# caomw/3DFeatureMatcher

Measured on AMD Instinct MI355X. Metric: matched+triangulated+normal-optimised keypoints/sec; HBM GB/s vs roofline, higher is better.
Workload: dtype f64

## Files before the change

### 3dfeaturematcher_amd/__init__.py

```python
from __future__ import annotations

import ctypes
import os

import numpy as np

_HERE = os.path.dirname(os.path.abspath(__file__))
LIB_PATH = os.environ.get("FM3D_LIB") or os.path.join(_HERE, "libfm3d.so")

FM3D_OK = 0
ERR_INVALID, ERR_HIP, ERR_UNSUPPORTED, ERR_NOMEM, ERR_PARSE, ERR_NAN_PLANE = -1, -2, -3, -4, -5, -6
FEAT_SURF, FEAT_ORB, FEAT_SIFT, FEAT_FAST, FEAT_STAR, FEAT_BRISK, FEAT_FREAK, FEAT_MSER, FEAT_OTHER = 0, 1, 2, 3, 4, 5, 6, 7, -1
DESC_F32, DESC_U8, DESC_BITS = 0, 1, 2
ST_OK, ST_NO_PIXELS, ST_ABORT_BBOX, ST_ABORT_PIX1, ST_ABORT_PIX2, ST_NAN_PLANE, ST_NAN_NORMAL = range(7)

EXPORTS = (
    "fm3d_settings_default", "fm3d_settings_load", "fm3d_settings_lookup", "fm3d_ctx_create", "fm3d_ctx_destroy", "fm3d_last_error",
    "fm3d_ctx_set_stream", "fm3d_knn2", "fm3d_match_nndr", "fm3d_setg12", "fm3d_g12_from_poses",
    "fm3d_camera2_from_g12", "fm3d_set_g12", "fm3d_get_camera2", "fm3d_triangulate", "fm3d_set_images",
    "fm3d_get_pyramid_level", "fm3d_optimize_normals", "fm3d_pipeline_upload", "fm3d_pipeline_run",
    "fm3d_records_download", "fm3d_pyrdown", "fm3d_neighborhood", "fm3d_undistort", "fm3d_version",
    "fm3d_gravity", "fm3d_features_frames", "fm3d_patch_size", "fm3d_export_patches", "fm3d_square_neighborhoods",
    "fm3d_circular_neighborhoods", "fm3d_surf_detect", "fm3d_surf_compute", "fm3d_extract_descriptors_from_patches", "fm3d_extract_descriptors_from_patches_any", "fm3d_pipeline_run_dlt", "fm3d_pipeline_dlt_download", "fm3d_pipeline_run_ncc",
    "fm3d_pipeline_ncc_download",
# ... 96 lines not shown
                     ("octave", "<i4"), ("class_id", "<i4")])
RECORD = np.dtype([("queryIdx", "<i4"), ("trainIdx", "<i4"), ("distance", "<f4"), ("status", "<i4"),
                   ("point", "<f8", (3,)), ("normal", "<f8", (3,))])


class LMStats(ctypes.Structure):
    _fields_ = [("points_in", ctypes.c_int64), ("points_kept", ctypes.c_int64), ("evaluations", ctypes.c_int64),
                ("pixel_evaluations", ctypes.c_int64), ("drops", ctypes.c_int64 * 8), ("kernel_ms", ctypes.c_double),
                ("groups", ctypes.c_int64), ("passes", ctypes.c_int64), ("cycles_terms", ctypes.c_int64),
                ("cycles_chain", ctypes.c_int64), ("cycles_control", ctypes.c_int64), ("cycles_total", ctypes.c_int64),
                ("wall_ticks_sum", ctypes.c_int64), ("wall_ticks_max", ctypes.c_int64),
                ("wall_clock_khz", ctypes.c_int64), ("class_passes", ctypes.c_int64 * 4),
                ("class_cycles", ctypes.c_int64 * 4), ("last_group_start_ticks", ctypes.c_int64),
                ("last_group_end_ticks", ctypes.c_int64), ("cycles_wait", ctypes.c_int64),
                ("chain_rounds", ctypes.c_int64), ("chain_chunks", ctypes.c_int64),
                ("queue_empty_ticks", ctypes.c_int64)]

    def as_dict(self):
        d = {k: getattr(self, k) for k, _ in self._fields_}
        for k in ("drops", "class_passes", "class_cycles"):
            d[k] = list(d[k])
        return d


class PipelineStats(ctypes.Structure):
    _fields_ = [("queries", ctypes.c_int64), ("trains", ctypes.c_int64), ("matches", ctypes.c_int64),
                ("inliers", ctypes.c_int64), ("kept", ctypes.c_int64), ("match_ms", ctypes.c_double),
                ("nndr_ms", ctypes.c_double), ("triangulate_ms", ctypes.c_double), ("pyramid_ms", ctypes.c_double),
                ("lm_ms", ctypes.c_double), ("total_ms", ctypes.c_double), ("lm", LMStats)]

    def as_dict(self):
        d = {k: getattr(self, k) for k, _ in self._fields_ if k != "lm"}
        d["lm"] = self.lm.as_dict()
        return d

# ... 1500 lines not shown
```

### 3dfeaturematcher_amd/csrc/fm3d_ctx.h

```cpp
#pragma once

#include <hip/hip_runtime.h>

#include <cstdint>
#include <cstdlib>
#include <string>
#include <vector>

#include "fm3d.h"
#include "fm3d_algebra.h"
#include "fm3d_kernels.h"

namespace fm3d_host {

inline bool poison_word(uint32_t* word) {
    const char* e = getenv("FM3D_DEBUG_POISON");
    if (!e || !e[0]) return false;
    *word = (uint32_t)strtoul(e, nullptr, 0);
    return true;
}
inline void poison_host(void* p, size_t n, uint32_t word) {
    uint8_t* b = (uint8_t*)p;
    for (size_t i = 0; i < n; i++) b[i] = (uint8_t)(word >> (8 * (i & 3)));
}
// ... 68 lines not shown
        uint32_t word;
        if (poison_word(&word)) poison_host(p, n, word);
        return hipSuccess;
    }
};
using DevBuf = Buf<DeviceMem>;
using HostBuf = Buf<PinnedMem>;

constexpr size_t kGuard(int w) { return (size_t)4 * w + 64; }
constexpr int kColStride(int h) { return (h + 2 + 63) / 64 * 64; }
constexpr size_t kColBytes(int w, int h) { return (size_t)(w + 2) * kColStride(h) + 64; }

struct PipeSmall {
    int32_t cnt[4];
    unsigned long long prob[2];
    unsigned long long lm[26];
};

struct KnnWork {
    DevBuf cq, ct;
    DevBuf q8, t8;
    DevBuf partIdx, partKey;
    DevBuf pairs;
    DevBuf idx, key, fkey;
};

enum class PairState { Idle, Full, MemberFront, DltFront, Ncc, Verified, DltVerified };

enum class Need { Idle, StagedIdle, Full, Dlt, Ncc, Verified, DltVerified };

enum Ev {
// ... 177 lines not shown
```

### 3dfeaturematcher_amd/csrc/fm3d_kernels.h

```cpp
#pragma once

#include <hip/hip_runtime.h>
#include <stdint.h>

#include "fm3d.h"
#include "fm3d_device.h"

#ifndef FM3D_RAY_AOS
#define FM3D_RAY_AOS 1
#endif

namespace fm3d {

struct LevelDesc {
    const uint8_t* img1;
    const uint8_t* img2;
    int w, h;
    const uint8_t* img2t;
    int hs;
};

struct ProjConst {
    double R[9], t[3];
    Camera cam;
// ... 37 lines not shown
    double* normals_;
    int* status_;
    int* info_;
    int* nfev_;
    int* mdat_;
    unsigned long long* statEval;
    unsigned long long* statPix;
    long long maxIter;
    long long maxTicks;
    int* overflow;
    int coop;
    int safe;
    unsigned long long* statPass;
    int nProb;
    const LMProblem* prob;
};
constexpr int kLMMaxProblems = 4;

constexpr int kLMRunning = 0x100;

constexpr int kLM2Slots = 15;
constexpr int kLM2Ring = 8;
constexpr int kLM2Threads = 64 * (kLM2Slots + 1);
template <bool MULTI, bool TREE, bool COLS>
__global__ void lm2_kernel(LMParams p);

struct KnnOut {
    int* idx;
    int* key;
    float* fkey;
};

// ... 375 lines not shown
```

### 3dfeaturematcher_amd/csrc/fm3d_lm.cpp

```cpp
#include <cmath>
#include <cstdlib>
#include <cstring>
#include <vector>

#include "fm3d_ctx.h"

using fm3d::LevelDesc;

using namespace fm3d_host;

namespace fm3d_host {

void fill_lm_cycles(const fm3d_ctx* c, const unsigned long long* cnt, fm3d_lm_stats* st) {
    st->groups = c->lmGroups;
    st->passes = (int64_t)cnt[3];
    st->cycles_terms = (int64_t)cnt[4];
    st->cycles_chain = (int64_t)cnt[5];
    st->cycles_control = (int64_t)cnt[6];
    st->cycles_total = (int64_t)cnt[7];
    st->wall_ticks_sum = (int64_t)cnt[8];
    st->wall_ticks_max = (int64_t)cnt[9];
    st->wall_clock_khz = c->wallKhz;
    for (int k = 0; k < 4; k++) {
        st->class_passes[k] = (int64_t)cnt[10 + k];
        st->class_cycles[k] = (int64_t)cnt[14 + k];
    }
    st->last_group_start_ticks = (int64_t)(cnt[18] - cnt[20]);
    st->last_group_end_ticks = (int64_t)(cnt[19] - cnt[20]);
    st->cycles_wait = (int64_t)cnt[24];
    st->chain_rounds = (int64_t)cnt[21];
    st->chain_chunks = (int64_t)cnt[22];
    st->queue_empty_ticks = cnt[25] ? (int64_t)(cnt[25] - cnt[20]) : 0;
}

fm3d::Camera lm_camera(const fm3d::Camera& cam) {
    fm3d::Camera k = cam;
    if (k.cx == 0.) k.cx = 0.;
    if (k.cy == 0.) k.cy = 0.;
    return k;
}

int lm_groups(fm3d_ctx* c, const void* kptr, int slots, long Ptot, long* out) {
    long groups = c->s.lmWaves;
    if (groups <= 0) {
        int cus = 0, perCU = 0;
        HIPCHK(c, hipDeviceGetAttribute(&cus, hipDeviceAttributeMultiprocessorCount, c->device));
        HIPCHK(c, hipOccupancyMaxActiveBlocksPerMultiprocessor(&perCU, kptr, fm3d::kLM2Threads, 0));
// ... 48 lines not shown
        if (q != c && (q->device != c->device || q->s.pyramids != levels || q->s.pixelsRay != c->s.pixelsRay ||
                       std::memcmp(&q->cam, &c->cam, sizeof(c->cam)) != 0 || q->s.boundWidth != c->s.boundWidth ||
                       q->s.boundHeight != c->s.boundHeight || q->s.zThresholdMax != c->s.zThresholdMax ||
                       q->s.epsilonLMMIN != c->s.epsilonLMMIN || q->s.lmReduction != c->s.lmReduction))
            return fail(c, FM3D_ERR_INVALID, "linked contexts need one device, camera and LM settings");
        const int P = src[j].P;
        HIPCHK(c, q->lmNormals.ensure((size_t)(P + 1) * 3 * sizeof(double)));
        HIPCHK(c, q->lmStatus.ensure((size_t)(P + 1) * sizeof(int)));
        HIPCHK(c, q->lmInfo.ensure((size_t)(P + 1) * 8 * sizeof(int)));
        HIPCHK(c, q->lmNfev.ensure((size_t)(P + 1) * 8 * sizeof(int)));
        HIPCHK(c, q->lmMdat.ensure((size_t)(P + 1) * sizeof(int)));
        HIPCHK(c, q->pcnt.ensure(64));
        Ptot += P;
    }
    HIPCHK(c, c->lmQueue.ensure(64 * sizeof(int)));
    HIPCHK(c, c->lmStat.ensure(256));
    if (c->s.lmReduction != 0 && c->s.lmReduction != 1)
        return fail(c, FM3D_ERR_INVALID, "lmReduction must be 0 (pixel order) or 1 (tree)");
    const bool tree = c->s.lmReduction != 0;
    const int slots = fm3d::kLM2Slots + (tree ? 1 : 0);
    bool multiPose = false;
    for (int j = 1; j < nProb; j++)
        multiPose |= std::memcmp(src[j].c->R2, src[0].c->R2, sizeof(c->R2)) != 0 ||
                     std::memcmp(src[j].c->t2, src[0].c->t2, sizeof(c->t2)) != 0;
    bool cols = true;
    for (int j = 0; j < nProb; j++) cols &= lm_prefers_cols(src[j].c);
    if (const char* lay = getenv("FM3D_LM_IMG2")) {
        if (!std::strcmp(lay, "rows")) cols = false;
        else if (!std::strcmp(lay, "cols")) cols = true;
        else if (std::strcmp(lay, "auto")) return fail(c, FM3D_ERR_INVALID, "FM3D_LM_IMG2 must be rows, cols or auto");
    }
// ... 78 lines not shown
    c->lmGroups = groups;
    {
        const long long perSlot = (Ptot + groups * slots - 1) / (groups * slots) + 1;
        p.maxIter = perSlot * (long long)(levels + 1) * 1600 + 10000;
        int khz = 0;
        if (hipDeviceGetAttribute(&khz, hipDeviceAttributeWallClockRate, c->device) != hipSuccess || khz <= 0) khz = 100000;
        const char* ms = getenv("FM3D_LM_MAX_SECONDS");
        const double secs = ms && atof(ms) > 0 ? atof(ms) : 300.;
        p.maxTicks = (long long)((double)khz * 1000. * secs);
        c->wallKhz = khz;
        const char* co = getenv("FM3D_LM_COOP");
        p.coop = co ? atoi(co) : 1;
        if (tree) p.coop = 0;
        const char* sf = getenv("FM3D_LM_SAFE");
        p.safe = sf ? atoi(sf) : 0;
    }
    {
        fm3d::LMReset rz{};
        rz.stat = c->lmStat.as<unsigned long long>();
        rz.queue = Ptot > 0 ? c->lmQueue.as<int>() : nullptr;
        rz.nProb = nProb;
        for (int j = 0; j < nProb; j++) {
            fm3d_ctx* q = src[j].c;
            rz.pcnt16[j] = q->pcnt.as<int>() + 4;
            rz.status[j] = q->lmStatus.as<int>();
            rz.info[j] = q->lmInfo.as<int>();
            rz.nfev[j] = q->lmNfev.as<int>();
            rz.P[j] = Ptot > 0 && src[j].P > 0 ? src[j].P : 0;
        }
        if (Ptot > 0) HIPCHK(c, hipEventRecord(e0, c->stream));
// ... 18 lines not shown
}

}

extern "C" {

int fm3d_optimize_normals(fm3d_ctx* c, double* points, int P, double* normals, int32_t* status, int32_t* info,
                          int32_t* nfev, int* nKept, fm3d_lm_stats* stats) {
    if (!c || !nKept || P < 0 || (P && (!points || !normals))) return fail(c, FM3D_ERR_INVALID, "bad argument");
    hipSetDevice(c->device);
    int r;
    if ((r = upload(c, c->pts, points, (size_t)P * 3 * sizeof(double)))) return r;
    if ((r = run_lm(c, P, nullptr, stats, c->ev[EV_LM_START], c->ev[EV_END]))) return r;
    std::vector<double> nrm((size_t)P * 3);
    std::vector<int> st(P), inf((size_t)P * 8), nf((size_t)P * 8);
    unsigned long long cnt[26] = {};
    if (P) {
        HIPCHK(c, hipMemcpyAsync(nrm.data(), c->lmNormals.p, nrm.size() * sizeof(double), hipMemcpyDeviceToHost, c->stream));
        HIPCHK(c, hipMemcpyAsync(st.data(), c->lmStatus.p, st.size() * sizeof(int), hipMemcpyDeviceToHost, c->stream));
        HIPCHK(c, hipMemcpyAsync(inf.data(), c->lmInfo.p, inf.size() * sizeof(int), hipMemcpyDeviceToHost, c->stream));
        HIPCHK(c, hipMemcpyAsync(nf.data(), c->lmNfev.p, nf.size() * sizeof(int), hipMemcpyDeviceToHost, c->stream));
        HIPCHK(c, hipMemcpyAsync(cnt, c->lmStat.p, sizeof(cnt), hipMemcpyDeviceToHost, c->stream));
    }
    HIPCHK(c, hipStreamSynchronize(c->stream));
    int overflow = 0;
    HIPCHK(c, hipMemcpy(&overflow, c->lmStat.as<unsigned long long>() + 2, sizeof(int), hipMemcpyDeviceToHost));
    if (overflow) return fail(c, FM3D_ERR_HIP, "LM kernel iteration guard tripped (internal error)");
    float ms = 0.f;
    if (P) hipEventElapsedTime(&ms, c->ev[EV_LM_START], c->ev[EV_END]);
    int kept = 0;
    bool nanPlane = false;
// ... 31 lines not shown
```

### 3dfeaturematcher_amd/csrc/fm3d_lm2.hip

```cpp
#include <hip/hip_runtime.h>
#include <float.h>
#include <stdint.h>

#include <type_traits>

#include "fm3d_device.h"
#include "fm3d_fastdiv.h"
#include "fm3d_kernels.h"
#include "fm3d_lmdif.h"

namespace fm3d {

namespace {

using namespace lmdif;

constexpr int kW = kLM2Slots;
constexpr int kWA = kW + 1;
constexpr int kE = 64;
constexpr int kR = kLM2Ring;
static_assert((kR & (kR - 1)) == 0, "ring depth: a power of two");
constexpr int kRow = kE + 2;
constexpr int kRS = (2 * kLM2Slots * kRow * 8 + 255) / 256 * 256 / 8;
#ifndef FM3D_EVAL_PIPE
#define FM3D_EVAL_PIPE 1
#endif

enum PassKind2 { Q_IDLE = 0, Q_INIT, Q_LEVEL, Q_EVAL, Q_QR1, Q_QR2, Q_QR3, Q_GRAM, Q_DONE };
enum SumKind { S_NONE = 0, S_ENORM, S_DOT };

typedef __attribute__((address_space(1))) double gdouble;
typedef __attribute__((address_space(1))) float gfloat;
typedef double d2v __attribute__((ext_vector_type(2)));
typedef __attribute__((address_space(1))) d2v gd2v;
typedef __attribute__((address_space(1))) int gint;
typedef __attribute__((address_space(1))) const long long gi64;
typedef __attribute__((address_space(1))) const uint8_t gu8;
// ... 23 lines not shown
    int pidx, m, L, i1ok, ekind, t0, q0, t1, bNaN;
};

struct PassOut2 {
    double nrm[2];
    double sum[2];
    double aqs1;
    double sq[2], g[3];
    int cnt, fail[2], ph3[2], i1fail, slow;
};

struct PassDesc {
    int nChunks, id;
    int kind[2];
    double agiant;
};

struct Slab {
    gdouble* RX;
    gdouble* RY;
    gfloat* I1;
    gfloat* DF;
    gfloat* DJ0;
    gfloat* DJ1;
    gint* KI;
};
template <int NS>
__device__ inline Slab slab_of(const LMParams& p, long gslot) {
    const size_t n = (size_t)p.nOffPad, G = (size_t)p.nWaves * NS;
    Slab s;
// ... 416 lines not shown
            }
        } else if (ps == Q_GRAM) {
            S.s.acnorm[0] = o.nrm[0];
            S.s.acnorm[1] = o.nrm[1];
            start_qr_tree(S, P, o);
        } else if (ps == Q_QR3) {
            const double tq1 = -o.sum[0] / S.usecond;
            finalize_qr(S, P, S.wa4s + S.usecond * tq1);
        }
    }
};

struct Shared {
    alignas(256) double ring[kR][kRS];
    int rowTag[kWA][kR];
    int consumed[kWA][2];
    int resultId[kWA][2];
    double result[kWA][2];
    Enorm chainEn[64];
    int done[kWA];
    int exited;
    int helper[kWA];
    int annSeq[kWA];
    int annBase[kWA], annId[kWA];
    int helpDone[kWA];
    int hfail[kWA][2], hph3[kWA][2];
    int hAtt[kWA], hSeen[kWA], hAnn[kWA];
    struct WaveStat {
        unsigned long long cnt[4], cyc[4], terms, ctl, wait, nPass, iter, t0;
    } ws[kWA];
// ... 51 lines not shown
    add(v1);
    add(v2);
    add(v3);
    return sum;
}

__device__ __forceinline__ int rfl(int v) { return __builtin_amdgcn_readfirstlane(v); }
__device__ __forceinline__ unsigned long long rfl_u64(unsigned long long v) {
    return ((unsigned long long)(unsigned)rfl((int)(v >> 32)) << 32) | (unsigned)rfl((int)v);
}
__device__ __forceinline__ const uint8_t* rfl_ptr(const uint8_t* q) {
    const unsigned long long v = (unsigned long long)q;
    return (const uint8_t*)(((unsigned long long)(unsigned)rfl((int)(v >> 32)) << 32) | (unsigned)rfl((int)v));
}

struct Producer {
    Shared* sh;
    int w, lane, me;
    int cmin;
    unsigned long long deadline;

    __device__ __forceinline__ void reserve(int c) {
        if (c >= cmin + kR) {
            cmin = rfl(min(lds_load_acq(&sh->consumed[w][0]), lds_load_acq(&sh->consumed[w][1])));
            if (c >= cmin + kR) {
                const long long c0 = clock64();
                do {
                    __builtin_amdgcn_s_sleep(1);
                    cmin = rfl(min(lds_load_acq(&sh->consumed[w][0]), lds_load_acq(&sh->consumed[w][1])));
                } while (c >= cmin + kR && wall_clock64() < deadline);
                const unsigned long long dt = clock64() - c0;
                if (lane == 0) sh->ws[me].wait += dt;
            }
        }
    }
    template <bool TWO = true>
    __device__ __forceinline__ void write(int c, double t0, double t1, int slowBits) {
        const int pos = c & (kR - 1);
        double* row0 = &sh->ring[pos][2 * w * kRow];
        row0[lane] = t0;
        if (TWO) row0[kRow + lane] = t1;
#if FM3D_TAG_NOWAIT
        __hip_atomic_store(&sh->rowTag[w][pos], (c << 2) | slowBits, __ATOMIC_RELAXED, __HIP_MEMORY_SCOPE_WORKGROUP);
#else
        __builtin_amdgcn_s_waitcnt(0xc07f);
        lds_store_rel(&sh->rowTag[w][pos], (c << 2) | slowBits);
#endif
    }
    template <bool TWO = true>
    __device__ __forceinline__ void put(int c, double t0, double t1, int slowBits) {
        reserve(c);
        write<TWO>(c, t0, t1, slowBits);
    }
#ifndef FM3D_SLOW_BRANCH
#define FM3D_SLOW_BRANCH 1
#endif
    template <bool TWO = true>
    __device__ __forceinline__ void write_terms(int c, double t0, double v0, bool slow0, double t1, double v1,
                                                bool slow1) {
#if FM3D_SLOW_BRANCH
        const int pos = c & (kR - 1);
        double* row0 = &sh->ring[pos][2 * w * kRow];
        row0[lane] = t0;
        if (TWO) row0[kRow + lane] = t1;
        int slowBits = 0;
        if (slow0 || (TWO && slow1)) {
            asm volatile("" ::: "memory");
            if (slow0) row0[lane] = v0;
            if (TWO && slow1) row0[kRow + lane] = v1;
            slowBits = (slow0 ? 1 : 0) | ((TWO && slow1) ? 2 : 0);
        }
        __builtin_amdgcn_s_waitcnt(0xc07f);
        lds_store_rel(&sh->rowTag[w][pos], (c << 2) | slowBits);
#else
        write<TWO>(c, slow0 ? v0 : t0, slow1 ? v1 : t1, (slow0 ? 1 : 0) | (slow1 ? 2 : 0));
#endif
    }
};

typedef __attribute__((address_space(4))) const ProjConst cProjConst;

__device__ __forceinline__ const cProjConst* proj_consts(const ProjConst* p) {
    int z;
    asm volatile("s_mov_b32 %0, 0" : "=s"(z));
    return (const cProjConst*)((const __attribute__((address_space(4))) char*)p + z);
}
__device__ __forceinline__ const cProjConst* proj_consts(const ProjConst* p, unsigned off) {
    unsigned z;
    asm volatile("s_mov_b32 %0, %1" : "=s"(z) : "s"(off));
    return (const cProjConst*)((const __attribute__((address_space(4))) char*)p + z);
}
// ... 94 lines not shown

__device__ __forceinline__ double chain_slow(int lane, double acc0, const double* row) {
    Enorm en = g_sh.chainEn[lane];
    en.s2 = acc0;
    for (int i = 0; i < kE; i++) en.add(row[i]);
    g_sh.chainEn[lane] = en;
    return en.s2;
}
__device__ __forceinline__ double chain_finish(int lane, double acc) {
    Enorm en = g_sh.chainEn[lane];
    en.s2 = acc;
    return en.finish();
}

__device__ __noinline__ void chain_wave(int lane, unsigned long long tStart, long long maxTicks,
                                        unsigned long long* statBusy, unsigned long long* statRounds) {
    __builtin_amdgcn_s_setprio(3);
    const int s = lane >> 1, which = lane & 1;
    bool alive = s < kW;
    const int ss_ = alive ? s : 0;
    int cur = 0, rem = 0, kind = S_NONE, pid = 0;
    bool inPass = false;
    double acc = 0.;
    unsigned long long busy = 0, tLast = 0, rounds = 0, chunks = 0;
    bool wasBusy = false;
    for (;;) {
        if ((long long)(wall_clock64() - tStart) > maxTicks) break;
        if (!__any(alive)) break;
#ifndef FM3D_CHAIN_ONETRIP
#define FM3D_CHAIN_ONETRIP 1
#endif
#if FM3D_CHAIN_ONETRIP
        auto tagRel = [&](int b) {
            return alive ? __hip_atomic_load(&g_sh.rowTag[ss_][(cur + b) & (kR - 1)], __ATOMIC_RELAXED, __HIP_MEMORY_SCOPE_WORKGROUP) : -1;
        };
        const int tag0 = tagRel(0), tg1 = tagRel(1), tg2 = tagRel(2), tg3 = tagRel(3);
        __builtin_amdgcn_fence(__ATOMIC_ACQUIRE, "workgroup");
#else
        const int tag0 = alive ? lds_load_acq(&g_sh.rowTag[ss_][cur & (kR - 1)]) : -1;
#endif
        const bool have = (tag0 >> 2) == cur;
        if (have && !inPass) {
            const PassDesc& d = g_sh.pd[ss_];
            rem = d.nChunks;
            kind = d.kind[which];
            pid = d.id;
            Enorm& en = g_sh.chainEn[lane];
            en.init(1);
            en.agiant = d.agiant;
            acc = 0.;
            inPass = true;
        }
        if (__any(have)) {
            const unsigned long long t = clock64();
            if (wasBusy) busy += t - tLast;
            tLast = t;
            wasBusy = true;
#ifndef FM3D_CHAIN_NB
#define FM3D_CHAIN_NB 4
#endif
#if FM3D_CHAIN_NB == 4
#if FM3D_CHAIN_ONETRIP
            const int tag1 = (have && rem >= 2) ? tg1 : -1, tag2 = (have && rem >= 3) ? tg2 : -1;
            const int tag3 = (have && rem >= 4) ? tg3 : -1;
#else
            const int tag1 = (have && rem >= 2) ? __hip_atomic_load(&g_sh.rowTag[ss_][(cur + 1) & (kR - 1)], __ATOMIC_RELAXED, __HIP_MEMORY_SCOPE_WORKGROUP) : -1;
            const int tag2 = (have && rem >= 3) ? __hip_atomic_load(&g_sh.rowTag[ss_][(cur + 2) & (kR - 1)], __ATOMIC_RELAXED, __HIP_MEMORY_SCOPE_WORKGROUP) : -1;
            const int tag3 = (have && rem >= 4) ? __hip_atomic_load(&g_sh.rowTag[ss_][(cur + 3) & (kR - 1)], __ATOMIC_RELAXED, __HIP_MEMORY_SCOPE_WORKGROUP) : -1;
            __builtin_amdgcn_fence(__ATOMIC_ACQUIRE, "workgroup");
#endif
            int nb = have ? 1 : 0;
            if (nb == 1 && (tag1 >> 2) == cur + 1) nb = 2;
            if (nb == 2 && (tag2 >> 2) == cur + 2) nb = 3;
            if (nb == 3 && (tag3 >> 2) == cur + 3) nb = 4;
            const int slowm = (tag0 & 3) | ((tag1 & 3) << 2) | ((tag2 & 3) << 4) | ((tag3 & 3) << 6);
#else
            const int tag1 = (have && rem >= 2) ? lds_load_acq(&g_sh.rowTag[ss_][(cur + 1) & (kR - 1)]) : -1;
            const int nb = have ? (((tag1 >> 2) == cur + 1) ? 2 : 1) : 0;
#endif
            rounds++;
            chunks += nb;
#pragma nounroll
            for (int b = 0; b < FM3D_CHAIN_NB; b++) {
                if (b < nb) {
                    const double* row = &g_sh.ring[cur & (kR - 1)][lane * kRow];
#if FM3D_CHAIN_NB == 4
                    const bool slow = ((slowm >> (2 * b + which)) & 1) != 0;
#else
                    const bool slow = (((b ? tag1 : tag0) >> which) & 1) != 0;
#endif
                    const double acc0 = acc;
                    acc = chain_sum64(acc, row);
                    if (kind == S_ENORM && slow) acc = chain_slow(lane, acc0, row);
                    cur++;
                    rem--;
                }
            }
            if (nb > 0) lds_store_rel(&g_sh.consumed[ss_][which], cur);
            if (have && rem == 0) {
                g_sh.result[ss_][which] = kind == S_ENORM ? chain_finish(lane, acc) : acc;
                lds_store_rel(&g_sh.resultId[ss_][which], pid);
                inPass = false;
            }
        } else {
            if (wasBusy) {
                busy += clock64() - tLast;
                wasBusy = false;
            }
            if (alive && !inPass && lds_load_acq(&g_sh.done[ss_])) alive = false;
            __builtin_amdgcn_s_sleep(1);
        }
    }
    if (lane == 0) {
        atomicAdd(statBusy, busy);
        atomicAdd(statRounds, rounds);
    }
    for (int o = 32; o > 0; o >>= 1) chunks += __shfl_xor(chunks, o);
    if (lane == 0) atomicAdd(statRounds + 1, chunks);
}

}

template <bool MULTI, bool TREE, bool COLS>
__global__ __launch_bounds__(kLM2Threads, 4) void lm2_kernel(LMParams p) {
    Shared& sh = g_sh;
    constexpr int NS = TREE ? kWA : kW;
    const int tid = threadIdx.x, lane = tid & 63, wave = tid >> 6;
    const unsigned long long tStart = wall_clock64(), cyStart = clock64();
    if (tid == 0) {
        sh.P = p;
        sh.exited = 0;
    }
    if (tid < NS) {
        for (int k = 0; k < kR; k++) sh.rowTag[tid][k] = -1;
        sh.consumed[tid][0] = sh.consumed[tid][1] = 0;
        sh.resultId[tid][0] = sh.resultId[tid][1] = 0;
        sh.done[tid] = 0;
        sh.helper[tid] = sh.annSeq[tid] = sh.helpDone[tid] = 0;
        sh.hAtt[tid] = -2;
        sh.hSeen[tid] = sh.hAnn[tid] = 0;
    }
    __syncthreads();

    if (wave < NS) {
        const int w = rfl(wave);
        const long gslot = (long)blockIdx.x * NS + w;
        Ctl2& ctl = sh.ctl[w];

        if (lane == 0) {
// ... 139 lines not shown
                    if (lane == 0) WS.nPass++;
                    cbase = chunkSeq;
                    chunkSeq = cbase + nCh;
                    k0 = 0;
                    kS = (p.coop && rfl(lds_load_acq(&sh.helper[w])) != 0) ? 2 : 1;
                }
                cbase = rfl(cbase);
                k0 = rfl(k0);
                kS = rfl(kS);
                const unsigned s8 = (unsigned)(((size_t)blockIdx.x * NS + tw) * p.nOffPad * 8);
                const int ekind = rfl(SP.ekind);
                const int nev = rfl(SP.nev);
                const bool jac = pass == Q_EVAL && ekind == E_JAC;
                cls = jac ? 0 : (pass == Q_EVAL ? 1 : 2);
                const double agiant = SP.agiant;
                if (!TREE && own && lane == 0) {
                    PassDesc& d = sh.pd[w];
                    d.nChunks = nCh;
                    d.id = passId;
                    d.agiant = agiant;
                    d.kind[0] = (pass == Q_QR1 || pass == Q_QR3) ? S_DOT : S_ENORM;
                    d.kind[1] = pass == Q_QR1 ? S_DOT : ((pass == Q_EVAL && nev == 2) ? S_ENORM : S_NONE);
                    if (kS == 2) {
                        sh.annBase[w] = cbase;
                        sh.annId[w] = passId;
                        lds_store_rel(&sh.annSeq[w], ++sh.hAnn[w]);
                    }
                }
                int fail0 = 0x7fffffff, fail1 = 0x7fffffff;
                int ph30 = 0, ph31 = 0;
                double aqs1 = 0.;
                double ta0 = 0., ta1 = 0., ta2 = 0., ta3 = 0., ta4 = 0.;
                bool tslow0 = false, tslow1 = false;
                if (pass == Q_EVAL) {
                    const double n00 = SP.n0[0], n10 = SP.n1[0], n20 = SP.n2[0], mm0 = SP.mm[0], w0 = SP.w[0];
                    const double n01 = SP.n0[1], n11 = SP.n1[1], n21 = SP.n2[1], mm1 = SP.mm[1], w1 = SP.w[1];
                    const double h0 = SP.hj[0], h1 = SP.hj[1], wF = SP.wF;
// ... 481 lines not shown
                                if (kc < nCh) {
                                    const Terms T = (kc == 0 || kc == nCh - 1) ? chunk(buf[j], kc, std::true_type())
                                                                               : chunk(buf[j], kc, std::false_type());
                                    if constexpr (TREE) {
                                        ta0 += T.t0;
                                        if (KIND == Q_QR1 || KIND == Q_GRAM) ta1 += T.t1;
                                        if (KIND == Q_GRAM) {
                                            ta2 += T.g0;
                                            ta3 += T.g1;
                                            ta4 += T.g2;
                                            tslow1 |= T.slow1;
                                        }
                                        tslow0 |= T.slow;
                                    } else {
                                        prod.reserve(cbase + kc);
                                        prod.write_terms<KIND == Q_QR1>(cbase + kc, T.t0, T.a, T.slow, T.t1, 0., false);
                                    }
                                    buf[j] = load(o4);
                                }
                                o4 += st4;
                            }
                        }
                    };
                    if (TREE && pass == Q_GRAM) {
                        if constexpr (TREE) {
                            if (fast)
                                run(std::integral_constant<int, Q_GRAM>(), std::true_type());
                            else
                                run(std::integral_constant<int, Q_GRAM>(), std::false_type());
                        }
                    } else if (fast) {
// ... 97 lines not shown
        }
        if (lane == 0) {
            lds_store_rel(&sh.done[w], 1);
            atomicAdd(p.statEval, (unsigned long long)ctl.cnt_eval);
            atomicAdd(p.statPix, (unsigned long long)ctl.cnt_pix);
            atomicAdd(p.statPass + 0, WS.nPass);
            atomicAdd(p.statPass + 1, WS.terms);
            atomicAdd(p.statPass + 3, WS.ctl);
            for (int k = 0; k < 4; k++) {
                atomicAdd(p.statPass + 7 + k, WS.cnt[k]);
                atomicAdd(p.statPass + 11 + k, WS.cyc[k]);
            }
            atomicAdd(p.statPass + 21, WS.wait);
        }
    } else {
        chain_wave(lane, tStart, p.maxTicks, p.statPass + 2, p.statPass + 18);
    }
    bool lastWave = false;
    if (lane == 0) lastWave = TREE ? atomicAdd(&sh.exited, 1) == NS - 1 : wave == kW;
    if (lastWave) {
        atomicAdd(p.statPass + 4, clock64() - cyStart);
        const unsigned long long wt = wall_clock64() - tStart;
        atomicAdd(p.statPass + 5, wt);
        atomicMax(p.statPass + 6, wt);
        atomicMax(p.statPass + 15, tStart);
        atomicMax(p.statPass + 16, wall_clock64());
        atomicMin(p.statPass + 17, tStart);
    }
}

template __global__ void lm2_kernel<false, false, false>(LMParams p);
// ... 10 lines not shown
```

### 3dfeaturematcher_amd/csrc/fm3d_misc.hip

```cpp
#include <hip/hip_runtime.h>
#include <stdint.h>

#include "fm3d_kernels.h"

namespace fm3d {

namespace {

template <int P, int Q>
__device__ __forceinline__ bool jacobi_pair(double* A, double* V) {
    double alpha = 0, beta = 0, gamma = 0;
#pragma unroll
    for (int i = 0; i < 4; i++) {
        double ap = A[i * 4 + P], aq = A[i * 4 + Q];
        alpha += ap * ap;
        beta += aq * aq;
        gamma += ap * aq;
    }
    if (gamma != 0. && fabs(gamma) > 1e-15 * sqrt(alpha * beta)) {
        double zeta = (beta - alpha) / (2. * gamma);
        double t = (zeta >= 0. ? 1. : -1.) / (fabs(zeta) + sqrt(1. + zeta * zeta));
        double cs = 1. / sqrt(1. + t * t);
        double sn = cs * t;
#pragma unroll
// ... 95 lines not shown
        out[3 * o + 2] = X[2] / X[3];
        srcIdx[o] = i;
    }
    if (lane == 0 && bid == (int)gridDim.x - 1) {
        const int total = ex + __popcll(bal);
        *count = total;
        if (hostCnt) {
            __hip_atomic_store(&hostCnt[0], p.Kdev ? *p.Kdev : p.K, __ATOMIC_RELAXED, __HIP_MEMORY_SCOPE_SYSTEM);
            __hip_atomic_store(&hostCnt[1], total, __ATOMIC_RELAXED, __HIP_MEMORY_SCOPE_SYSTEM);
        }
    }
}

__global__ void lm_reset_kernel(LMReset r, int maxP) {
    const int t = blockIdx.x * blockDim.x + threadIdx.x;
    if (t < 32) r.stat[t] = t == 20 ? ~0ull : 0ull;
    if (r.queue && t < 64) r.queue[t] = 0;
    for (int j = 0; j < r.nProb; j++) {
        if (t < 4) r.pcnt16[j][t] = 0;
        if (t < r.P[j]) r.status[j][t] = kLMRunning;
        if (t < 8 * r.P[j]) {
            r.info[j][t] = 0;
            r.nfev[j][t] = 0;
        }
    }
    (void)maxP;
}

__device__ inline int reflect101(int q, int len) {
    if (len == 1) return 0;
    while (q < 0 || q >= len) q = q < 0 ? -q : 2 * len - q - 2;
// ... 399 lines not shown
```

### 3dfeaturematcher_amd/csrc/fm3d_pipeline.cpp

```cpp
#include <cstdlib>
#include <cstring>
#include <vector>

#include "fm3d_ctx.h"
#include "fm3d_internal.h"

using namespace fm3d_host;

namespace {

int require(fm3d_ctx* c, Need need) {
    if (need == Need::StagedIdle && (!c || !c->staged)) return fail(c, FM3D_ERR_INVALID, "fm3d_pipeline_upload not called");
    if (!c) return FM3D_ERR_INVALID;
    const PairState s = c->pipe.state;
    if (need != Need::StagedIdle && need != Need::Idle) {
        if (s == PairState::Verified && need != Need::Verified)
            return fail(c, FM3D_ERR_INVALID, "a verified frame pair is pending: fm3d_pipeline_wait_verified");
        if (s == PairState::DltVerified && need != Need::DltVerified)
            return fail(c, FM3D_ERR_INVALID, "a verified front half is pending: fm3d_pipeline_wait_dlt_verified");
    }
    if (need == Need::Verified && s != PairState::Verified)
        return fail(c, FM3D_ERR_INVALID, "no verified frame pair submitted (fm3d_pipeline_submit_verified)");
    if (need == Need::DltVerified && s != PairState::DltVerified)
        return fail(c, FM3D_ERR_INVALID, "no verified front half submitted (fm3d_pipeline_submit_dlt_verified)");
// ... 164 lines not shown
    return enqueue_normals(c, out, ls);
}

int enqueue_linked(fm3d_ctx* c, const std::vector<fm3d_ctx*>& ms, fm3d_lm_stats* ls) {
    int r;
    if ((r = pipeline_front(c))) return r;
    std::vector<LMSrc> src;
    for (fm3d_ctx* m : ms) {
        HIPCHK(c, hipStreamWaitEvent(c->stream, m->pipe.evFront, 0));
        src.push_back({m, m->pipe.nA, m->pcnt.as<int>() + 1});
        HIPCHK(c, hipEventRecord(m->ev[EV_NORMAL_START], c->stream));
    }
    src.push_back({c, c->pipe.nA, c->pcnt.as<int>() + 1});
    if ((r = run_lm_multi(c, src.data(), (int)src.size(), ls, c->ev[EV_NORMAL_START], c->ev[EV_NORMAL_END]))) return r;
    for (fm3d_ctx* m : ms) {
        HIPCHK(m, m->lmStat.ensure(256));
        HIPCHK(c, hipMemcpyAsync(m->lmStat.p, c->lmStat.p, sizeof(PipeSmall::lm), hipMemcpyDeviceToDevice, c->stream));
    }
    HIPCHK(c, hipEventRecord(c->pipe.evLm, c->stream));
    if ((r = enqueue_epilogue(c, c->pipe.subOut, c->lmStat.p))) return r;
    for (fm3d_ctx* m : ms) {
        HIPCHK(c, hipEventRecord(m->ev[EV_NORMAL_END], c->stream));
        m->pipe.subLm = *ls;
        m->lmGroups = c->lmGroups;
        m->wallKhz = c->wallKhz;
        hipSetDevice(m->device);
        HIPCHK(m, hipStreamWaitEvent(m->stream, c->pipe.evLm, 0));
        if ((r = enqueue_epilogue(m, m->pipe.subOut, m->lmStat.p))) return r;
        m->pipe.state = PairState::Full;
    }
    return FM3D_OK;
// ... 510 lines not shown
```

### include/fm3d.h

```cpp
#ifndef FM3D_H
#define FM3D_H

#include <stdint.h>

#ifdef __cplusplus
extern "C" {
#endif

#define FM3D_OK 0
#define FM3D_ERR_INVALID (-1)
#define FM3D_ERR_HIP (-2)
#define FM3D_ERR_UNSUPPORTED (-3)
#define FM3D_ERR_NOMEM (-4)
#define FM3D_ERR_PARSE (-5)
#define FM3D_ERR_NAN_PLANE (-6)

#define FM3D_ST_OK 0
#define FM3D_ST_NO_PIXELS 1
#define FM3D_ST_ABORT_BBOX 2
#define FM3D_ST_ABORT_PIX1 3
#define FM3D_ST_ABORT_PIX2 4
#define FM3D_ST_NAN_PLANE 5
#define FM3D_ST_NAN_NORMAL 6

// ... 81 lines not shown
    int64_t points_in;
    int64_t points_kept;
    int64_t evaluations;
    int64_t pixel_evaluations;
    int64_t drops[8];
    double kernel_ms;
    int64_t groups;
    int64_t passes;
    int64_t cycles_terms, cycles_chain, cycles_control, cycles_total;
    int64_t wall_ticks_sum, wall_ticks_max, wall_clock_khz;
    int64_t class_passes[4], class_cycles[4];
    int64_t last_group_start_ticks, last_group_end_ticks;
    int64_t cycles_wait;
    int64_t chain_rounds, chain_chunks;
    int64_t queue_empty_ticks;
} fm3d_lm_stats;

typedef struct fm3d_pipeline_stats {
    int64_t queries, trains, matches, inliers, kept;
    double match_ms, nndr_ms, triangulate_ms, pyramid_ms, lm_ms, total_ms;
    fm3d_lm_stats lm;
} fm3d_pipeline_stats;

int fm3d_settings_default(fm3d_settings *s);
int fm3d_settings_load(const char *path, fm3d_settings *s);
int fm3d_settings_lookup(const char *path, const char *key, char *out, int cap, int *len);
int fm3d_ctx_create(const fm3d_settings *s, int device, fm3d_ctx **out);
void fm3d_ctx_destroy(fm3d_ctx *ctx);
const char *fm3d_last_error(const fm3d_ctx *ctx);
int fm3d_ctx_set_stream(fm3d_ctx *ctx, void *hip_stream);
// ... 294 lines not shown
```

Before: 37570.

## Add opt-in exact wave-reduced chunk summaries so the chain can skip serial sums

Producer waves can now precompute an exact wave-level sum of each 64-term chunk, using DPP adds on values rounded to a binade grid taken from the chain's current accumulator exponent. They also store a validity window alongside it. The chain wave then accepts a chunk with a single add when the accumulator lies in that window, and falls back to the ordered 64-term sum otherwise, so results stay bit-identical while the serial dependence chain shrinks. The path is gated by FM3D_LM_RSUM and stays off by default (auto maps to 0). Changes that apply regardless of the flag: ring rows are padded from 66 to 70 doubles to stagger LDS banks, row tags carry 4 flag bits instead of 2, and new per-class fast/slow counters are added to the stats.

```diff
diff --git a/3dfeaturematcher_amd/__init__.py b/3dfeaturematcher_amd/__init__.py
--- a/3dfeaturematcher_amd/__init__.py
+++ b/3dfeaturematcher_amd/__init__.py
@@ -134,11 +134,12 @@
                 ("class_cycles", ctypes.c_int64 * 4), ("last_group_start_ticks", ctypes.c_int64),
                 ("last_group_end_ticks", ctypes.c_int64), ("cycles_wait", ctypes.c_int64),
                 ("chain_rounds", ctypes.c_int64), ("chain_chunks", ctypes.c_int64),
-                ("queue_empty_ticks", ctypes.c_int64)]
+                ("queue_empty_ticks", ctypes.c_int64), ("rsum_fast", ctypes.c_int64 * 4),
+                ("rsum_slow", ctypes.c_int64 * 4)]
 
     def as_dict(self):
         d = {k: getattr(self, k) for k, _ in self._fields_}
-        for k in ("drops", "class_passes", "class_cycles"):
+        for k in ("drops", "class_passes", "class_cycles", "rsum_fast", "rsum_slow"):
             d[k] = list(d[k])
         return d
 
diff --git a/3dfeaturematcher_amd/csrc/fm3d_ctx.h b/3dfeaturematcher_amd/csrc/fm3d_ctx.h
--- a/3dfeaturematcher_amd/csrc/fm3d_ctx.h
+++ b/3dfeaturematcher_amd/csrc/fm3d_ctx.h
@@ -106,7 +106,7 @@
 struct PipeSmall {
     int32_t cnt[4];
     unsigned long long prob[2];
-    unsigned long long lm[26];
+    unsigned long long lm[34];
 };
 
 struct KnnWork {
diff --git a/3dfeaturematcher_amd/csrc/fm3d_kernels.h b/3dfeaturematcher_amd/csrc/fm3d_kernels.h
--- a/3dfeaturematcher_amd/csrc/fm3d_kernels.h
+++ b/3dfeaturematcher_amd/csrc/fm3d_kernels.h
@@ -75,8 +75,10 @@
     unsigned long long* statPass;
     int nProb;
     const LMProblem* prob;
+    int rsum;
 };
 constexpr int kLMMaxProblems = 4;
+constexpr int kLMRsumAuto = 0;
 
 constexpr int kLMRunning = 0x100;
 
diff --git a/3dfeaturematcher_amd/csrc/fm3d_lm.cpp b/3dfeaturematcher_amd/csrc/fm3d_lm.cpp
--- a/3dfeaturematcher_amd/csrc/fm3d_lm.cpp
+++ b/3dfeaturematcher_amd/csrc/fm3d_lm.cpp
@@ -31,6 +31,10 @@
     st->chain_rounds = (int64_t)cnt[21];
     st->chain_chunks = (int64_t)cnt[22];
     st->queue_empty_ticks = cnt[25] ? (int64_t)(cnt[25] - cnt[20]) : 0;
+    for (int k = 0; k < 4; k++) {
+        st->rsum_fast[k] = (int64_t)cnt[26 + 2 * k];
+        st->rsum_slow[k] = (int64_t)cnt[27 + 2 * k];
+    }
 }
 
 fm3d::Camera lm_camera(const fm3d::Camera& cam) {
@@ -109,7 +113,7 @@
         Ptot += P;
     }
     HIPCHK(c, c->lmQueue.ensure(64 * sizeof(int)));
-    HIPCHK(c, c->lmStat.ensure(256));
+    HIPCHK(c, c->lmStat.ensure(512));
     if (c->s.lmReduction != 0 && c->s.lmReduction != 1)
         return fail(c, FM3D_ERR_INVALID, "lmReduction must be 0 (pixel order) or 1 (tree)");
     const bool tree = c->s.lmReduction != 0;
@@ -218,6 +222,13 @@
         if (tree) p.coop = 0;
         const char* sf = getenv("FM3D_LM_SAFE");
         p.safe = sf ? atoi(sf) : 0;
+        p.rsum = fm3d::kLMRsumAuto;
+        if (const char* rs = getenv("FM3D_LM_RSUM")) {
+            if (!std::strcmp(rs, "0")) p.rsum = 0;
+            else if (!std::strcmp(rs, "1")) p.rsum = 15;
+            else if (std::strcmp(rs, "auto")) return fail(c, FM3D_ERR_INVALID, "FM3D_LM_RSUM must be 0, 1 or auto");
+        }
+        if (p.safe || tree) p.rsum = 0;
     }
     {
         fm3d::LMReset rz{};
@@ -266,7 +277,7 @@
     if ((r = run_lm(c, P, nullptr, stats, c->ev[EV_LM_START], c->ev[EV_END]))) return r;
     std::vector<double> nrm((size_t)P * 3);
     std::vector<int> st(P), inf((size_t)P * 8), nf((size_t)P * 8);
-    unsigned long long cnt[26] = {};
+    unsigned long long cnt[34] = {};
     if (P) {
         HIPCHK(c, hipMemcpyAsync(nrm.data(), c->lmNormals.p, nrm.size() * sizeof(double), hipMemcpyDeviceToHost, c->stream));
         HIPCHK(c, hipMemcpyAsync(st.data(), c->lmStatus.p, st.size() * sizeof(int), hipMemcpyDeviceToHost, c->stream));
diff --git a/3dfeaturematcher_amd/csrc/fm3d_lm2.hip b/3dfeaturematcher_amd/csrc/fm3d_lm2.hip
--- a/3dfeaturematcher_amd/csrc/fm3d_lm2.hip
+++ b/3dfeaturematcher_amd/csrc/fm3d_lm2.hip
@@ -8,6 +8,7 @@
 #include "fm3d_fastdiv.h"
 #include "fm3d_kernels.h"
 #include "fm3d_lmdif.h"
+#include "fm3d_rsum.h"
 
 namespace fm3d {
 
@@ -20,7 +21,8 @@
 constexpr int kE = 64;
 constexpr int kR = kLM2Ring;
 static_assert((kR & (kR - 1)) == 0, "ring depth: a power of two");
-constexpr int kRow = kE + 2;
+constexpr int kRow = kE + 6;
+static_assert(kRow % 2 == 0 && (kRow / 2) % 2 == 1, "ring rows: 16 B times an odd number apart");
 constexpr int kRS = (2 * kLM2Slots * kRow * 8 + 255) / 256 * 256 / 8;
 #ifndef FM3D_EVAL_PIPE
 #define FM3D_EVAL_PIPE 1
@@ -74,6 +76,7 @@
     int nChunks, id;
     int kind[2];
     double agiant;
+    int rs[2];
 };
 
 struct Slab {
@@ -520,6 +523,8 @@
 struct Shared {
     alignas(256) double ring[kR][kRS];
     int rowTag[kWA][kR];
+    int predHi[kWA][2];
+    unsigned long long rsCnt[8];
     int consumed[kWA][2];
     int resultId[kWA][2];
     double result[kWA][2];
@@ -601,6 +606,25 @@
     return (const uint8_t*)(((unsigned long long)(unsigned)rfl((int)(v >> 32)) << 32) | (unsigned)rfl((int)v));
 }
 
+__device__ __forceinline__ int tag_of(int c, int flags) { return (int)(((unsigned)c << 4) | (unsigned)flags); }
+__device__ __forceinline__ bool tag_is(int tag, int c) { return ((unsigned)tag >> 4) == ((unsigned)c & 0x0fffffffu); }
+
+template <int CTRL, int ROWS = 0xf>
+__device__ __forceinline__ double dpp_add(double x) {
+    const int lo = __builtin_amdgcn_update_dpp(0, __double2loint(x), CTRL, ROWS, 0xf, false);
+    const int hi = __builtin_amdgcn_update_dpp(0, __double2hiint(x), CTRL, ROWS, 0xf, false);
+    return x + __hiloint2double(hi, lo);
+}
+__device__ __forceinline__ double wave_sum_exact(double x) {
+    x = dpp_add<0xB1>(x);
+    x = dpp_add<0x4E>(x);
+    x = dpp_add<0x141>(x);
+    x = dpp_add<0x140>(x);
+    x = dpp_add<0x142, 0xa>(x);
+    x = dpp_add<0x143, 0xc>(x);
+    return x;
+}
+
 struct Producer {
     Shared* sh;
     int w, lane, me;
@@ -628,10 +652,10 @@
         row0[lane] = t0;
         if (TWO) row0[kRow + lane] = t1;
 #if FM3D_TAG_NOWAIT
-        __hip_atomic_store(&sh->rowTag[w][pos], (c << 2) | slowBits, __ATOMIC_RELAXED, __HIP_MEMORY_SCOPE_WORKGROUP);
+        __hip_atomic_store(&sh->rowTag[w][pos], tag_of(c, slowBits), __ATOMIC_RELAXED, __HIP_MEMORY_SCOPE_WORKGROUP);
 #else
         __builtin_amdgcn_s_waitcnt(0xc07f);
-        lds_store_rel(&sh->rowTag[w][pos], (c << 2) | slowBits);
+        lds_store_rel(&sh->rowTag[w][pos], tag_of(c, slowBits));
 #endif
     }
     template <bool TWO = true>
@@ -658,10 +682,48 @@
             slowBits = (slow0 ? 1 : 0) | ((TWO && slow1) ? 2 : 0);
         }
         __builtin_amdgcn_s_waitcnt(0xc07f);
-        lds_store_rel(&sh->rowTag[w][pos], (c << 2) | slowBits);
+        lds_store_rel(&sh->rowTag[w][pos], tag_of(c, slowBits));
 #else
         write<TWO>(c, slow0 ? v0 : t0, slow1 ? v1 : t1, (slow0 ? 1 : 0) | (slow1 ? 2 : 0));
 #endif
+    }
+    template <bool TWO, bool ENORM>
+    __device__ __forceinline__ void write_terms_rs(int c, double t0, double v0, bool slow0, double t1, bool rs0,
+                                                   bool rs1) {
+        const int pos = c & (kR - 1);
+        double* row0 = &sh->ring[pos][2 * w * kRow];
+        row0[lane] = t0;
+        if (TWO) row0[kRow + lane] = t1;
+        int flags = 0;
+        if (slow0) {
+            asm volatile("" ::: "memory");
+            row0[lane] = v0;
+            flags = 1;
+        }
+        auto summary = [&](double t, int k, bool enorm) {
+            const int hi = rfl(__hip_atomic_load(&sh->predHi[w][k], __ATOMIC_RELAXED, __HIP_MEMORY_SCOPE_WORKGROUP));
+            RsumBin b;
+            const bool bok = rsum_bin(rsum_exp_of_hi(hi), b);
+            bool bad;
+            const double r = rsum_step(b, t, bad);
+            if (bok && __ballot(bad) == 0) {
+                const double R = wave_sum_exact(r);
+                const double A = enorm ? R : wave_sum_exact(fabs(r));
+                double lo, hi;
+                const bool wok = rsum_window(b.M, A, lo, hi);
+                if (lane == 63) {
+                    double* sm = row0 + k * kRow + kE;
+                    sm[0] = R;
+                    sm[1] = lo;
+                    sm[2] = hi;
+                }
+                if ((__ballot(wok) >> 63) & 1) flags |= 4 << k;
+            }
+        };
+        if (rs0 && !slow0) summary(t0, 0, ENORM);
+        if (TWO && rs1) summary(t1, 1, false);
+        __builtin_amdgcn_s_waitcnt(0xc07f);
+        lds_store_rel(&sh->rowTag[w][pos], tag_of(c, flags));
     }
 };
 
@@ -786,12 +848,15 @@
 }
 
 __device__ __noinline__ void chain_wave(int lane, unsigned long long tStart, long long maxTicks,
-                                        unsigned long long* statBusy, unsigned long long* statRounds) {
+                                        unsigned long long* statBusy, unsigned long long* statRounds, int rsum,
+                                        unsigned long long* statRs) {
     __builtin_amdgcn_s_setprio(3);
     const int s = lane >> 1, which = lane & 1;
     bool alive = s < kW;
     const int ss_ = alive ? s : 0;
     int cur = 0, rem = 0, kind = S_NONE, pid = 0;
+    int rsIdx = 0;
+    unsigned pFast = 0, pSlow = 0;
     bool inPass = false;
     double acc = 0.;
     unsigned long long busy = 0, tLast = 0, rounds = 0, chunks = 0;
@@ -807,16 +872,26 @@
             return alive ? __hip_atomic_load(&g_sh.rowTag[ss_][(cur + b) & (kR - 1)], __ATOMIC_RELAXED, __HIP_MEMORY_SCOPE_WORKGROUP) : -1;
         };
         const int tag0 = tagRel(0), tg1 = tagRel(1), tg2 = tagRel(2), tg3 = tagRel(3);
+        int tg4 = -1, tg5 = -1, tg6 = -1, tg7 = -1;
+        static_assert(kR == 8, "the chain reads eight tags");
+        if (rsum) {
+            tg4 = tagRel(4);
+            tg5 = tagRel(5);
+            tg6 = tagRel(6);
+            tg7 = tagRel(7);
+        }
         __builtin_amdgcn_fence(__ATOMIC_ACQUIRE, "workgroup");
 #else
         const int tag0 = alive ? lds_load_acq(&g_sh.rowTag[ss_][cur & (kR - 1)]) : -1;
 #endif
-        const bool have = (tag0 >> 2) == cur;
+        const bool have = tag_is(tag0, cur);
         if (have && !inPass) {
             const PassDesc& d = g_sh.pd[ss_];
             rem = d.nChunks;
             kind = d.kind[which];
             pid = d.id;
+            rsIdx = d.rs[which];
+            pFast = pSlow = 0;
             Enorm& en = g_sh.chainEn[lane];
             en.init(1);
             en.agiant = d.agiant;
@@ -842,16 +917,78 @@
             __builtin_amdgcn_fence(__ATOMIC_ACQUIRE, "workgroup");
 #endif
             int nb = have ? 1 : 0;
-            if (nb == 1 && (tag1 >> 2) == cur + 1) nb = 2;
-            if (nb == 2 && (tag2 >> 2) == cur + 2) nb = 3;
-            if (nb == 3 && (tag3 >> 2) == cur + 3) nb = 4;
+            if (nb == 1 && tag_is(tag1, cur + 1)) nb = 2;
+            if (nb == 2 && tag_is(tag2, cur + 2)) nb = 3;
+            if (nb == 3 && tag_is(tag3, cur + 3)) nb = 4;
             const int slowm = (tag0 & 3) | ((tag1 & 3) << 2) | ((tag2 & 3) << 4) | ((tag3 & 3) << 6);
 #else
             const int tag1 = (have && rem >= 2) ? lds_load_acq(&g_sh.rowTag[ss_][(cur + 1) & (kR - 1)]) : -1;
-            const int nb = have ? (((tag1 >> 2) == cur + 1) ? 2 : 1) : 0;
+            int nb = have ? (tag_is(tag1, cur + 1) ? 2 : 1) : 0;
 #endif
             rounds++;
-            chunks += nb;
+#if FM3D_CHAIN_NB == 4 && FM3D_CHAIN_ONETRIP
+            if (rsum) {
+                const int tgs[kR] = {tag0, tg1, tg2, tg3, tg4, tg5, tg6, tg7};
+                unsigned validm = 0, slowm8 = 0;
+                nb = 0;
+#pragma unroll
+                for (int b = 0; b < kR; b++) {
+                    if (have && nb == b && b < rem && tag_is(tgs[b], cur + b)) {
+                        nb = b + 1;
+                        validm |= (unsigned)((tgs[b] >> (2 + which)) & 1) << b;
+                        slowm8 |= (unsigned)((tgs[b] >> which) & 1) << b;
+                    }
+                }
+                if (kind == S_NONE) validm = 0xff;
+                int j = 0;
+#pragma nounroll
+                for (int step = 0; step <= 4; step++) {
+                    for (;;) {
+                        const bool tryFast = j < nb && ((validm >> j) & 1);
+                        bool ok = false;
+                        if (tryFast) {
+                            ok = kind == S_NONE;
+                            if (!ok) {
+                                const double* sm = &g_sh.ring[cur & (kR - 1)][lane * kRow + kE];
+                                const double2 rl = *reinterpret_cast<const double2*>(sm);
+                                double sNew = acc;
+                                ok = rsum_accept(sNew, rl.x, rl.y, sm[2]);
+                                acc = sNew;
+                            }
+                            if (ok) {
+                                cur++;
+                                rem--;
+                                j++;
+                                pFast++;
+                            } else {
+                                validm &= ~(1u << j);
+                            }
+                        }
+                        if (!__any(ok)) break;
+                    }
+                    const bool slowNow = step < 4 && j < nb;
+                    if (!__any(slowNow)) break;
+                    if (slowNow) {
+                        const double* row = &g_sh.ring[cur & (kR - 1)][lane * kRow];
+                        const double acc0 = acc;
+                        acc = chain_sum64(acc, row);
+                        if (kind == S_ENORM && ((slowm8 >> j) & 1)) acc = chain_slow(lane, acc0, row);
+                        cur++;
+                        rem--;
+                        j++;
+                        pSlow++;
+                    }
+                }
+                nb = j;
+                if (nb > 0)
+                    __hip_atomic_store(&g_sh.predHi[ss_][which], rsum_hi(acc), __ATOMIC_RELAXED, __HIP_MEMORY_SCOPE_WORKGROUP);
+                if (have && rem == 0 && rsIdx > 0) {
+                    atomicAdd(&g_sh.rsCnt[2 * (rsIdx - 1)], (unsigned long long)pFast);
+                    atomicAdd(&g_sh.rsCnt[2 * (rsIdx - 1) + 1], (unsigned long long)pSlow);
+                }
+            } else
+#endif
+            {
 #pragma nounroll
             for (int b = 0; b < FM3D_CHAIN_NB; b++) {
                 if (b < nb) {
@@ -868,6 +1005,8 @@
                     rem--;
                 }
             }
+            }
+            chunks += nb;
             if (nb > 0) lds_store_rel(&g_sh.consumed[ss_][which], cur);
             if (have && rem == 0) {
                 g_sh.result[ss_][which] = kind == S_ENORM ? chain_finish(lane, acc) : acc;
@@ -889,6 +1028,7 @@
     }
     for (int o = 32; o > 0; o >>= 1) chunks += __shfl_xor(chunks, o);
     if (lane == 0) atomicAdd(statRounds + 1, chunks);
+    if (rsum && lane < 8) atomicAdd(statRs + lane, g_sh.rsCnt[lane]);
 }
 
 }
@@ -902,9 +1042,11 @@
     if (tid == 0) {
         sh.P = p;
         sh.exited = 0;
+        for (int k = 0; k < 8; k++) sh.rsCnt[k] = 0;
     }
     if (tid < NS) {
         for (int k = 0; k < kR; k++) sh.rowTag[tid][k] = -1;
+        sh.predHi[tid][0] = sh.predHi[tid][1] = 0;
         sh.consumed[tid][0] = sh.consumed[tid][1] = 0;
         sh.resultId[tid][0] = sh.resultId[tid][1] = 0;
         sh.done[tid] = 0;
@@ -1074,6 +1216,9 @@
                 const bool jac = pass == Q_EVAL && ekind == E_JAC;
                 cls = jac ? 0 : (pass == Q_EVAL ? 1 : 2);
                 const double agiant = SP.agiant;
+                const int rsum = TREE ? 0 : rfl(p.rsum);
+                const bool rs0 = pass == Q_QR1 ? (rsum & 1) : pass == Q_QR2 ? (rsum & 4) : pass == Q_QR3 ? (rsum & 8) : 0;
+                const bool rs1 = pass == Q_QR1 && (rsum & 2);
                 if (!TREE && own && lane == 0) {
                     PassDesc& d = sh.pd[w];
                     d.nChunks = nCh;
@@ -1081,6 +1226,8 @@
                     d.agiant = agiant;
                     d.kind[0] = (pass == Q_QR1 || pass == Q_QR3) ? S_DOT : S_ENORM;
                     d.kind[1] = pass == Q_QR1 ? S_DOT : ((pass == Q_EVAL && nev == 2) ? S_ENORM : S_NONE);
+                    d.rs[0] = rs0 ? (pass == Q_QR1 ? 1 : pass == Q_QR2 ? 3 : 4) : 0;
+                    d.rs[1] = rs1 ? 2 : 0;
                     if (kS == 2) {
                         sh.annBase[w] = cbase;
                         sh.annId[w] = passId;
@@ -1592,7 +1739,11 @@
                                         tslow0 |= T.slow;
                                     } else {
                                         prod.reserve(cbase + kc);
-                                        prod.write_terms<KIND == Q_QR1>(cbase + kc, T.t0, T.a, T.slow, T.t1, 0., false);
+                                        if (rs0 || rs1)
+                                            prod.write_terms_rs<KIND == Q_QR1, KIND == Q_QR2>(cbase + kc, T.t0, T.a, T.slow, T.t1,
+                                                                                              rs0, rs1);
+                                        else
+                                            prod.write_terms<KIND == Q_QR1>(cbase + kc, T.t0, T.a, T.slow, T.t1, 0., false);
                                     }
                                     buf[j] = load(o4);
                                 }
@@ -1720,7 +1871,7 @@
             atomicAdd(p.statPass + 21, WS.wait);
         }
     } else {
-        chain_wave(lane, tStart, p.maxTicks, p.statPass + 2, p.statPass + 18);
+        chain_wave(lane, tStart, p.maxTicks, p.statPass + 2, p.statPass + 18, rfl(p.rsum), p.statPass + 23);
     }
     bool lastWave = false;
     if (lane == 0) lastWave = TREE ? atomicAdd(&sh.exited, 1) == NS - 1 : wave == kW;
diff --git a/3dfeaturematcher_amd/csrc/fm3d_misc.hip b/3dfeaturematcher_amd/csrc/fm3d_misc.hip
--- a/3dfeaturematcher_amd/csrc/fm3d_misc.hip
+++ b/3dfeaturematcher_amd/csrc/fm3d_misc.hip
@@ -133,7 +133,7 @@
 
 __global__ void lm_reset_kernel(LMReset r, int maxP) {
     const int t = blockIdx.x * blockDim.x + threadIdx.x;
-    if (t < 32) r.stat[t] = t == 20 ? ~0ull : 0ull;
+    if (t < 40) r.stat[t] = t == 20 ? ~0ull : 0ull;
     if (r.queue && t < 64) r.queue[t] = 0;
     for (int j = 0; j < r.nProb; j++) {
         if (t < 4) r.pcnt16[j][t] = 0;
diff --git a/3dfeaturematcher_amd/csrc/fm3d_pipeline.cpp b/3dfeaturematcher_amd/csrc/fm3d_pipeline.cpp
--- a/3dfeaturematcher_amd/csrc/fm3d_pipeline.cpp
+++ b/3dfeaturematcher_amd/csrc/fm3d_pipeline.cpp
@@ -202,7 +202,7 @@
     src.push_back({c, c->pipe.nA, c->pcnt.as<int>() + 1});
     if ((r = run_lm_multi(c, src.data(), (int)src.size(), ls, c->ev[EV_NORMAL_START], c->ev[EV_NORMAL_END]))) return r;
     for (fm3d_ctx* m : ms) {
-        HIPCHK(m, m->lmStat.ensure(256));
+        HIPCHK(m, m->lmStat.ensure(512));
         HIPCHK(c, hipMemcpyAsync(m->lmStat.p, c->lmStat.p, sizeof(PipeSmall::lm), hipMemcpyDeviceToDevice, c->stream));
     }
     HIPCHK(c, hipEventRecord(c->pipe.evLm, c->stream));
diff --git a/3dfeaturematcher_amd/csrc/fm3d_rsum.h b/3dfeaturematcher_amd/csrc/fm3d_rsum.h
--- /dev/null
+++ b/3dfeaturematcher_amd/csrc/fm3d_rsum.h
@@ -0,0 +1,59 @@
+#pragma once
+#include <stdint.h>
+
+#if defined(__HIPCC__) || defined(__CUDACC__)
+#define FM3D_RSUM_HD __host__ __device__ inline
+#else
+#define FM3D_RSUM_HD inline
+#endif
+
+namespace fm3d {
+
+FM3D_RSUM_HD double rsum_from_hi(int hi) {
+    const uint64_t b = (uint64_t)(uint32_t)hi << 32;
+    double d;
+    __builtin_memcpy(&d, &b, 8);
+    return d;
+}
+FM3D_RSUM_HD int rsum_hi(double d) {
+    uint64_t b;
+    __builtin_memcpy(&b, &d, 8);
+    return (int)(uint32_t)(b >> 32);
+}
+FM3D_RSUM_HD int rsum_exp_of_hi(int hi) { return (hi >> 20) & 0x7ff; }
+
+struct RsumBin {
+    double M, half, hq;
+};
+FM3D_RSUM_HD bool rsum_bin(int be, RsumBin& b) {
+    const bool ok = be >= 64 && be <= 0x7fd;
+    const int e = ok ? be : 1023;
+    b.M = rsum_from_hi((e << 20) | 0x80000);
+    b.half = rsum_from_hi((e - 1) << 20);
+    b.hq = rsum_from_hi((e - 53) << 20);
+    return ok;
+}
+
+FM3D_RSUM_HD double rsum_step(const RsumBin& b, double t, bool& bad) {
+    const double r = (b.M + t) - b.M;
+    const double d = t - r;
+    bad = !(__builtin_fabs(t) < b.half) || __builtin_fabs(d) == b.hq;
+    return r;
+}
+
+FM3D_RSUM_HD bool rsum_window(double M, double A, double& lo, double& hi) {
+    const int e = rsum_exp_of_hi(rsum_hi(M));
+    const double b = rsum_from_hi(e << 20), q = rsum_from_hi((e - 52) << 20);
+    lo = (b + A) + q;
+    hi = ((b + b) - A) - q;
+    return A < b;
+}
+
+FM3D_RSUM_HD bool rsum_accept(double& S, double R, double lo, double hi) {
+    const double aS = __builtin_fabs(S);
+    if (!(aS >= lo && aS < hi)) return false;
+    S = S + R;
+    return true;
+}
+
+}
diff --git a/include/fm3d.h b/include/fm3d.h
--- a/include/fm3d.h
+++ b/include/fm3d.h
@@ -119,6 +119,7 @@
     int64_t cycles_wait;
     int64_t chain_rounds, chain_chunks;
     int64_t queue_empty_ticks;
+    int64_t rsum_fast[4], rsum_slow[4];
 } fm3d_lm_stats;
 
 typedef struct fm3d_pipeline_stats {
```

Measured after the change: 37650 (median of 6 runs). Within noise of the previous version (+0.2%).
